# quickwit-oss/quickwit

Hardware: AMD Instinct MI355X
Metric: leaf_search_docs_per_sec (higher is better)
Workload: dtype u32+f32; 1 GPU; 3term_bm25_or_100000000; query=body:w00009 OR body:w00010 OR body:w00011, docs_per_gpu=100000000, splits_per_gpu=1, max_hits=10, parallelism=split-dp1

## Files before the change

### include/quickwit_amd.h

```cpp
#ifndef QUICKWIT_AMD_H
#define QUICKWIT_AMD_H

#include <stddef.h>
#include <stdint.h>

#ifdef __cplusplus
extern "C" {
#endif

typedef struct qw_ctx qw_ctx;

typedef struct qw_buf {
    uint8_t* data;
    size_t len;
} qw_buf;

enum qw_status {
    QW_OK = 0,
    QW_ERR_INVALID_ARGUMENT = -1,
    QW_ERR_INVALID_QUERY = -2,
    QW_ERR_NOT_FOUND = -3,
    QW_ERR_INTERNAL = -4,
    QW_ERR_NO_GPU = -5,
    QW_ERR_BAD_SPLIT = -6,
    QW_ERR_OVER_MEMORY_BUDGET = -7,
};

qw_ctx* qw_ctx_create(const char* config_json);
void qw_ctx_free(qw_ctx* ctx);

int32_t qw_ctx_add_split(qw_ctx* ctx, const char* split_id,
                         const uint8_t* data, size_t len);
int32_t qw_ctx_remove_split(qw_ctx* ctx, const char* split_id);

int32_t qw_leaf_search(qw_ctx* ctx, const uint8_t* leaf_search_request_pb,
                       size_t len, qw_buf* response_pb_out);

void qw_buf_free(qw_buf* buf);

int32_t qw_fetch_docs(qw_ctx* ctx, const uint8_t* fetch_docs_request_pb,
                      size_t len, qw_buf* response_pb_out);

int32_t qw_leaf_list_terms(qw_ctx* ctx, const uint8_t* leaf_list_terms_request_pb,
                           size_t len, qw_buf* response_pb_out);

int32_t qw_merge_leaf_responses(const uint8_t* search_request_pb,
                                size_t search_request_len,
                                const uint8_t** response_pbs,
                                const size_t* response_lens, size_t n,
                                qw_buf* merged_out);

int32_t qw_finalize_agg_to_json(const uint8_t* blob, size_t len,
                                const char* agg_request_json,
                                qw_buf* json_out);

const char* qw_last_error(const qw_ctx* ctx);


int32_t qw_kernel_stats(qw_ctx* ctx, const char* kernel_name,
                        double* total_ms, uint64_t* launches);
void qw_kernel_stats_reset(qw_ctx* ctx);
int32_t qw_ctx_device_sync(qw_ctx* ctx);

int32_t qw_ctx_memory_stats(qw_ctx* ctx, uint64_t* used_bytes,
                            uint64_t* budget_bytes, uint64_t* splits_bytes);

int32_t qw_absence_cache_stats(qw_ctx* ctx, uint64_t* hits, uint64_t* misses,
                               uint64_t* entries);

const char* qw_version(void);

#ifdef __cplusplus
}
#endif

#endif
```

### quickwit_amd/api.py

```python
import ctypes
import json
import os

from . import proto

REPO_ROOT = os.path.dirname(os.path.dirname(os.path.abspath(__file__)))


class _Buf(ctypes.Structure):
    _fields_ = [("data", ctypes.POINTER(ctypes.c_uint8)), ("len", ctypes.c_size_t)]


def _bind(lib, syms):
    getattr(lib, syms["create"]).restype = ctypes.c_void_p
    getattr(lib, syms["add_split"]).argtypes = [
        ctypes.c_void_p, ctypes.c_char_p, ctypes.c_char_p, ctypes.c_size_t]
    getattr(lib, syms["leaf_search"]).argtypes = [
        ctypes.c_void_p, ctypes.c_char_p, ctypes.c_size_t, ctypes.POINTER(_Buf)]
    getattr(lib, syms["last_error"]).restype = ctypes.c_char_p
    getattr(lib, syms["last_error"]).argtypes = [ctypes.c_void_p]
    getattr(lib, syms["buf_free"]).argtypes = [ctypes.POINTER(_Buf)]


class _BaseSearcher:
# ... 98 lines not shown
        buf = _Buf()
        rc = fn(self._ctx, req_pb, len(req_pb), ctypes.byref(buf))
        if rc != 0:
            raise RuntimeError(f"fetch_docs failed ({rc}): {self._err()}")
        out = ctypes.string_at(buf.data, buf.len)
        self._lib.qw_buf_free(ctypes.byref(buf))
        return proto.decode("FetchDocsResponse", out)

    def leaf_list_terms(self, req: dict) -> dict:
        fn = self._lib.qw_leaf_list_terms
        fn.argtypes = [ctypes.c_void_p, ctypes.c_char_p, ctypes.c_size_t,
                       ctypes.POINTER(_Buf)]
        req_pb = proto.encode("LeafListTermsRequest", req)
        buf = _Buf()
        rc = fn(self._ctx, req_pb, len(req_pb), ctypes.byref(buf))
        if rc != 0:
            raise RuntimeError(f"leaf_list_terms failed ({rc}): {self._err()}")
        out = ctypes.string_at(buf.data, buf.len)
        self._lib.qw_buf_free(ctypes.byref(buf))
        return proto.decode("LeafListTermsResponse", out)

    def kernel_stats(self, name: str):
        fn = self._lib.qw_kernel_stats
        fn.argtypes = [ctypes.c_void_p, ctypes.c_char_p,
                       ctypes.POINTER(ctypes.c_double), ctypes.POINTER(ctypes.c_uint64)]
        ms = ctypes.c_double()
        n = ctypes.c_uint64()
        rc = fn(self._ctx, name.encode(), ctypes.byref(ms), ctypes.byref(n))
        if rc != 0:
            raise KeyError(name)
        return ms.value, n.value

    def kernel_stats_reset(self):
        self._lib.qw_kernel_stats_reset.argtypes = [ctypes.c_void_p]
        self._lib.qw_kernel_stats_reset(self._ctx)

    def memory_stats(self):
        fn = self._lib.qw_ctx_memory_stats
        fn.argtypes = [ctypes.c_void_p] + [ctypes.POINTER(ctypes.c_uint64)] * 3
        u, b, s = ctypes.c_uint64(), ctypes.c_uint64(), ctypes.c_uint64()
        rc = fn(self._ctx, ctypes.byref(u), ctypes.byref(b), ctypes.byref(s))
        if rc != 0:
            raise RuntimeError(f"memory_stats failed: {rc}")
        return u.value, b.value, s.value

    def absence_cache_stats(self):
        fn = self._lib.qw_absence_cache_stats
        fn.argtypes = [ctypes.c_void_p] + [ctypes.POINTER(ctypes.c_uint64)] * 3
        h, m, e = ctypes.c_uint64(), ctypes.c_uint64(), ctypes.c_uint64()
        rc = fn(self._ctx, ctypes.byref(h), ctypes.byref(m), ctypes.byref(e))
        if rc != 0:
            raise RuntimeError(f"absence_cache_stats failed: {rc}")
        return h.value, m.value, e.value

    def device_sync(self):
        self._lib.qw_ctx_device_sync.argtypes = [ctypes.c_void_p]
        rc = self._lib.qw_ctx_device_sync(self._ctx)
        if rc != 0:
            raise RuntimeError(f"device_sync failed: {self._err()}")


def make_leaf_request(query_ast: dict | str, schema: dict, splits: list,
                      max_hits: int = 10, sort_fields: list | None = None,
                      aggregation: dict | None = None, start_offset: int = 0,
                      start_timestamp: int | None = None,
                      end_timestamp: int | None = None) -> dict:
    sreq = {
        "index_id_patterns": ["bench-index"],
        "query_ast": query_ast if isinstance(query_ast, str) else json.dumps(query_ast),
        "max_hits": max_hits,
        "start_offset": start_offset,
    }
    if sort_fields:
        sreq["sort_fields"] = sort_fields
    if aggregation is not None:
        sreq["aggregation_request"] = json.dumps(aggregation)
    if start_timestamp is not None:
        sreq["start_timestamp"] = start_timestamp
    if end_timestamp is not None:
        sreq["end_timestamp"] = end_timestamp
    offsets = []
    for s in splits:
        if isinstance(s, dict):
            offsets.append(s)
            continue
        sid, ndocs = s[0], s[1]
        e = {"split_id": sid, "num_docs": ndocs}
        if len(s) > 2:
            e["split_footer_start"], e["split_footer_end"] = s[2], s[3]
        offsets.append(e)
    return {
        "search_request": sreq,
        "leaf_requests": [{"doc_mapper_ord": 0, "index_uri_ord": 0,
                           "split_offsets": offsets}],
        "doc_mappers": [json.dumps(schema)],
        "index_uris": ["ram:///bench-index"],
    }
```

### quickwit_amd/csrc/gpu_types.h

```cpp
#pragma once
#include <cstdint>

namespace qw {

#ifndef QW_TILE_DOCS
#define QW_TILE_DOCS 8192
#endif
constexpr uint32_t TILE_DOCS = QW_TILE_DOCS;
constexpr uint32_t TILE_THREADS = 256;
constexpr uint32_t KTAB_LDS_MAX = 4;
constexpr uint32_t AGG_LDS_BUCKETS = 2048;
constexpr uint32_t TOPK_BINS = 4096;

enum TermRole : uint32_t { ROLE_SHOULD = 0, ROLE_MUST = 1, ROLE_MUST_NOT = 2 };

struct TermDev {
    uint32_t role;
    uint32_t grp;
    uint32_t n_blocks;
    uint64_t skip_off;
    uint64_t payload_off;
    uint64_t norms_off;
    float weight;
    uint32_t ktab_idx;
// ... 62 lines not shown
    uint64_t sub_values_off[4];
    uint64_t sub_nulls_off[4];
    uint32_t sub_width[4];
    uint32_t sub_is_i64[4];
    uint32_t c_shift[4];
    uint32_t c_histo;
    uint32_t c_missing;
    double c_interval[4], c_offset[4];
    int64_t c_base[4];
    uint32_t p_si;
    uint64_t p_out;
    int32_t p_k_lo;
    uint32_t p_n_keys;
    uint64_t p_bound_off;
};

struct QueryDev {
    const uint8_t* split;
    const uint8_t* scratch;
    uint8_t* results;
    uint32_t num_docs;
    uint32_t n_tiles;
    uint32_t n_terms;
    uint32_t n_must;
    uint32_t n_must_not;
    uint32_t n_preds;
    uint32_t n_aggs;
    uint32_t msm;
    uint32_t scoring;
    uint32_t match_all;
    uint32_t collect_hits;
    uint32_t sort_asc;
    uint32_t wide_cand;
    uint32_t sort_src;
    uint32_t sort_width;
    uint64_t sort_values_off;
    uint64_t sort_nulls_off;
    uint32_t agg_fast;
    uint32_t agg_nt;
    uint32_t nt_decode;
    uint64_t bitmap_out;
    uint64_t terms_off;
    uint64_t preds_off;
    uint64_t aggs_off;
    uint64_t ktabs_off;
    uint32_t n_ktabs;
    uint32_t _pad_ktab;
    uint64_t norms_stage_off;
    uint64_t tile_counts_off;
    uint64_t cand_count_off;
    uint64_t cand_off;
    uint64_t cand_cap;
    uint64_t hist_off;
};

}
```

### quickwit_amd/csrc/kernels.hip

```cpp
#include <hip/hip_runtime.h>

#include "gpu_types.h"

namespace qw {

#pragma pack(push, 1)
struct SkipEntryDev {
    uint32_t first_doc;
    uint32_t last_doc;
    uint32_t word_off;
    uint8_t id_bits;
    uint8_t tf_bits;
    uint16_t count;
};
#pragma pack(pop)

__device__ __forceinline__ uint32_t lane_id() { return threadIdx.x & 63u; }

__device__ __forceinline__ uint64_t extract_bits(const uint32_t* base, uint64_t bitpos,
                                                 uint32_t w) {
    uint64_t word = bitpos >> 5;
    uint32_t sh = uint32_t(bitpos & 31);
    uint64_t v = (uint64_t(base[word]) | (uint64_t(base[word + 1]) << 32)) >> sh;
    return v & ((1ull << w) - 1ull);
}

__device__ __forceinline__ void extract_bits_pair(const uint32_t* base, uint32_t j,
                                                  uint32_t w, uint32_t* g0,
                                                  uint32_t* g1) {
    if (w <= 16) {
        uint64_t bitpos = uint64_t(j) * w;
        uint64_t word = bitpos >> 5;
        uint32_t sh = uint32_t(bitpos & 31);
        uint64_t v = (uint64_t(base[word]) | (uint64_t(base[word + 1]) << 32)) >> sh;
        uint32_t mask = (1u << w) - 1u;
        *g0 = uint32_t(v) & mask;
        *g1 = uint32_t(v >> w) & mask;
    } else {
        *g0 = uint32_t(extract_bits(base, uint64_t(j) * w, w));
        *g1 = uint32_t(extract_bits(base, uint64_t(j + 1) * w, w));
    }
}

__device__ __forceinline__ uint32_t wave_incl_scan_u32(uint32_t v) {
    #pragma unroll
    for (int d = 1; d < 64; d <<= 1) {
        uint32_t n = __shfl_up(v, d, 64);
        if ((threadIdx.x & 63u) >= uint32_t(d)) v += n;
    }
    return v;
}

__device__ __forceinline__ uint32_t f32_sortable(float f) {
    uint32_t b = __float_as_uint(f);
    return (b & 0x80000000u) ? ~b : (b | 0x80000000u);
}

__device__ __forceinline__ uint64_t f64_sortable(double d) {
    uint64_t b = __double_as_longlong(d);
    return (b & 0x8000000000000000ull) ? ~b : (b | 0x8000000000000000ull);
}

template <bool NS, bool NB, bool NA, bool NC>
struct SmemMap {
    static constexpr uint32_t score_off = 0;
    static constexpr uint32_t score_end = NS ? TILE_DOCS * 4 : 0;
    static constexpr uint32_t bits_acc_off = score_end;
    static constexpr uint32_t bits_not_off = bits_acc_off + (NB ? TILE_DOCS / 8 : 0);
    static constexpr uint32_t bits_end = bits_not_off + (NB ? TILE_DOCS / 8 : 0);
    static constexpr uint32_t bits_m_off = bits_end;
    static constexpr uint32_t word_pref_off = bits_m_off + (NC ? TILE_DOCS / 8 : 0);
    static constexpr uint32_t coll_end = word_pref_off + (NC ? TILE_DOCS / 8 : 0);
    static constexpr uint32_t agg_hist_off = coll_end;
    static constexpr uint32_t agg_terms_off = agg_hist_off + (NA ? AGG_LDS_BUCKETS * 4 : 0);
    static constexpr uint32_t agg_end = agg_terms_off + (NA ? AGG_LDS_BUCKETS * 4 : 0);
    static constexpr uint32_t tail_off = agg_end;
    static constexpr uint32_t total = tail_off + 4 * 4 + 4 * 4 + 4;
};

constexpr uint32_t tile_lds_bytes(bool ns, bool nb, bool na, bool nc) {
    return (ns ? TILE_DOCS * 4 : 0) + (nb ? 2 * TILE_DOCS / 8 : 0) +
           (nc ? 2 * TILE_DOCS / 8 : 0) + (na ? 2 * AGG_LDS_BUCKETS * 4 : 0) + 36;
}

template <bool SCORE>
__device__ void decode_term_tile(const QueryDev& q, const TermDev& t, uint32_t tile,
                                 uint32_t tile_lo, uint32_t tile_hi, float* score,
                                 uint32_t* bitset, bool scoring,
                                 const float* ktab_lds = nullptr,
                                 const uint8_t* norms_lds = nullptr) {
    const uint32_t* ranges = (const uint32_t*)t.ranges_addr;
    uint32_t blo = ranges[tile], bhi = ranges[q.n_tiles + tile];
    if (blo >= bhi) return;
    const SkipEntryDev* __restrict__ skip = (const SkipEntryDev*)(q.split + t.skip_off);
    const uint32_t* __restrict__ payload = (const uint32_t*)(q.split + t.payload_off);
    const uint8_t* __restrict__ norms = t.norms_off ? q.split + t.norms_off : nullptr;
    const bool nlds = norms_lds && t.norms_off &&
                      t.norms_off == q.norms_stage_off;
    const float* __restrict__ ktab =
        (ktab_lds ? ktab_lds : (const float*)(q.scratch + q.ktabs_off)) +
        256 * t.ktab_idx;
// ... 264 lines not shown
        else lo = mid + 1;
    }
    return lo + 1;
}

__device__ __forceinline__ uint64_t agg_ord(const QueryDev& q, uint64_t values_off,
                                            uint32_t width, uint32_t doc) {
    const uint8_t* col = q.split + values_off;
    switch (width) {
        case 1: return col[doc];
        case 2: return ((const uint16_t*)col)[doc];
        default: return ((const uint32_t*)col)[doc];
    }
}

__device__ __forceinline__ uint64_t wide_sort_key(const QueryDev& q, uint32_t d,
                                                  float sc) {
    if (q.sort_src == 0) return 0;
    if (q.sort_nulls_off) {
        const uint64_t* nulls = (const uint64_t*)(q.split + q.sort_nulls_off);
        if (!((nulls[d >> 6] >> (d & 63)) & 1)) return 0;
    }
    uint64_t S = 0;
    if (q.sort_src == 1) {
        S = uint64_t(f32_sortable(sc)) << 32;
    } else {
        const uint8_t* col = q.split + q.sort_values_off;
        switch (q.sort_width) {
            case 1: S = col[d]; break;
            case 2: S = ((const uint16_t*)col)[d]; break;
            case 4: S = ((const uint32_t*)col)[d]; break;
            default: S = ((const uint64_t*)col)[d]; break;
        }
        if (q.sort_src == 3) S ^= (1ull << 63);
        else if (q.sort_src == 4) S = f64_sortable(__longlong_as_double(S));
    }
    return q.sort_asc ? ~S : S;
}

__device__ __forceinline__ int64_t histo_bucket(const QueryDev& q, const AggDev& a,
                                                uint32_t doc) {
    if (a.int_fast) {
        const int64_t* col = (const int64_t*)(q.split + a.values_off);
        int64_t num = col[doc] - a.i_offset;
        int64_t idx = int64_t(floor(double(num) * a.inv_interval));
        if (idx * a.i_interval > num) --idx;
        else if ((idx + 1) * a.i_interval <= num) ++idx;
        return idx - a.base_index;
    }
    double v = agg_value(q, a.values_off, a.value_width, a.value_is_i64, doc);
    return int64_t(floor((v - a.offset) / a.interval)) - a.base_index;
}

template <bool NS, bool NB, bool NA, bool NC>
__global__ void __launch_bounds__(TILE_THREADS) k_leaf_tile_t(QueryDev q,
                                                              uint32_t tile_base,
                                                              uint32_t tile_end,
                                                              uint32_t do_count) {
    using M = SmemMap<NS, NB, NA, NC>;
    extern __shared__ uint8_t smem[];
    float* sc_score = (float*)(smem + M::score_off);
    uint32_t* sc_bits_acc = (uint32_t*)(smem + M::bits_acc_off);
    uint32_t* sc_bits_not = (uint32_t*)(smem + M::bits_not_off);
    uint32_t* sc_bits_m = (uint32_t*)(smem + M::bits_m_off);
    uint32_t* sc_word_pref = (uint32_t*)(smem + M::word_pref_off);
    uint32_t* sc_agg_hist = (uint32_t*)(smem + M::agg_hist_off);
    uint32_t* sc_agg_terms = (uint32_t*)(smem + M::agg_terms_off);
    uint32_t* sc_agg_matched = (uint32_t*)(smem + M::tail_off);
    uint32_t* sc_wave_base = sc_agg_matched + 4;
    uint32_t* sc_cand_base = sc_wave_base + 4;
    uint8_t* sc_norms = nullptr;
    float* sc_ktabs = nullptr;
    if (NS) {
        uint32_t soff = M::total;
        if (q.norms_stage_off) {
            sc_norms = smem + soff;
            soff += TILE_DOCS;
        }
        if (q.scoring && q.n_ktabs) {
            sc_ktabs = (float*)(smem + soff);
            const float* g = (const float*)(q.scratch + q.ktabs_off);
            for (uint32_t i = threadIdx.x; i < 256u * q.n_ktabs;
                 i += TILE_THREADS)
                sc_ktabs[i] = g[i];
        }
    }

    const TermDev* __restrict__ terms = (const TermDev*)(q.scratch + q.terms_off);
    const PredDev* __restrict__ preds = (const PredDev*)(q.scratch + q.preds_off);
    const AggDev* __restrict__ aggs = (const AggDev*)(q.scratch + q.aggs_off);
    uint32_t* tile_counts = (uint32_t*)(q.results + q.tile_counts_off);
    uint32_t* cand_count = (uint32_t*)(q.results + q.cand_count_off);
    uint64_t* cand = (uint64_t*)(q.results + q.cand_off);

    if (NA && q.n_aggs) {
        for (uint32_t i = threadIdx.x; i < AGG_LDS_BUCKETS; i += TILE_THREADS) {
            sc_agg_hist[i] = 0;
            sc_agg_terms[i] = 0;
        }
        if (threadIdx.x < 4) sc_agg_matched[threadIdx.x] = 0;
    }
    const int64_t* af_col = nullptr;
    const uint8_t* af_tcol = nullptr;
    int64_t af_ioff = 0, af_ivl = 1, af_base = 0;
    double af_inv = 0;
    uint32_t af_twidth = 0, af_hrep = 0, af_trep = 0, af_par = 0;
    bool af_terms = false;
// ... 358 lines not shown
                            if (a.lds_slot == 0)
                                atomicAdd(&sc_agg_hist[a.lds_rep == 2
                                                           ? uint32_t(idx) * 2 +
                                                                 (lane_id() & 1u)
                                                           : uint32_t(idx)],
                                          1u);
                            else
                                atomicAdd((unsigned long long*)(q.results + a.counts_out) +
                                              idx, 1ull);
                            for (uint32_t si = 0; si < a.n_sub; ++si) {
                                if (!a.sub_width[si]) continue;
                                if (a.sub_nulls_off[si]) {
                                    const uint64_t* sn =
                                        (const uint64_t*)(q.split + a.sub_nulls_off[si]);
                                    if (!((sn[d >> 6] >> (d & 63)) & 1)) continue;
                                }
                                double sv = agg_value(q, a.sub_values_off[si],
                                                      a.sub_width[si], a.sub_is_i64[si], d);
                                if (si == a.p_si) {
                                    uint32_t sj = perc_slot(q, a, sv);
                                    atomicAdd((unsigned long long*)(q.results +
                                                                    a.p_out) +
                                                  uint64_t(idx) *
                                                      (a.p_n_keys + 1) +
                                                  sj,
                                              1ull);
                                    continue;
                                }
                                uint8_t* slot = q.results + a.sub_out +
                                                (uint64_t(idx) * a.n_sub + si) * 40;
                                atomicAdd((unsigned long long*)slot, 1ull);
                                atomicAdd((double*)(slot + 8), sv);
                                atomicMin((unsigned long long*)(slot + 16),
                                          (unsigned long long)f64_sortable(sv));
                                atomicMax((unsigned long long*)(slot + 24),
                                          (unsigned long long)f64_sortable(sv));
                                atomicAdd((double*)(slot + 32), sv * sv);
                            }
                        }
                    }
            }
            if (NC) {
                uint64_t mb = __ballot(m);
                uint32_t wbase = (li - lane_id()) >> 5;
                if (lane_id() == 0) sc_bits_m[wbase] = uint32_t(mb);
                else if (lane_id() == 32) sc_bits_m[wbase + 1] = uint32_t(mb >> 32);
            }
        }
        if (NC && q.bitmap_out) {
            __syncthreads();
            ((uint32_t*)q.bitmap_out)[uint64_t(tile) * (TILE_DOCS / 32) +
                                      threadIdx.x] = sc_bits_m[threadIdx.x];
        }
        if (NC) {
            static_assert(TILE_DOCS == 32 * TILE_THREADS,
                          "collection assumes one 32-doc bitset word per thread");
            __syncthreads();
            uint32_t w = threadIdx.x;
            uint32_t cnt = __popc(sc_bits_m[w]);
            uint32_t incl = wave_incl_scan_u32(cnt);
            uint32_t wv = threadIdx.x >> 6;
            if (lane_id() == 63) sc_wave_base[wv] = incl;
            __syncthreads();
            uint32_t wave_off = 0;
            for (uint32_t i = 0; i < wv; ++i) wave_off += sc_wave_base[i];
            sc_word_pref[w] = wave_off + incl - cnt;
            uint32_t tile_total = sc_wave_base[0] + sc_wave_base[1] +
                                  sc_wave_base[2] + sc_wave_base[3];
            if (threadIdx.x == 0) {
                *sc_cand_base = atomicAdd(cand_count, tile_total);
                if (do_count) tile_counts[tile] = tile_total;
            }
            __syncthreads();
            uint64_t base = *sc_cand_base;
            {
                uint32_t wd = threadIdx.x;
                uint32_t bits = sc_bits_m[wd];
                uint64_t rank = sc_word_pref[wd];
                while (bits) {
                    uint32_t b = __ffs(bits) - 1u;
                    bits &= bits - 1u;
                    uint32_t li = wd * 32u + b;
                    uint32_t d = tile_lo + li;
                    float sc = (NS && q.scoring) ? sc_score[li] : 0.f;
                    uint64_t pos = base + rank++;
                    if (pos >= q.cand_cap) break;
                    if (q.wide_cand) {
                        uint64_t key = wide_sort_key(q, d, sc);
                        cand[2 * pos] = key;
                        cand[2 * pos + 1] =
                            (uint64_t(__float_as_uint(sc)) << 32) | d;
                    } else {
                        uint32_t kh = q.scoring ? f32_sortable(sc) : 0u;
                        if (q.sort_asc) kh = ~kh;
                        uint32_t kl = q.sort_asc ? ~d : d;
                        cand[pos] = (uint64_t(kh) << 32) | kl;
                    }
                }
            }
        } else if (do_count) {
            __syncthreads();
            #pragma unroll
            for (int dlt = 32; dlt; dlt >>= 1) local_count += __shfl_down(local_count, dlt, 64);
            if (lane_id() == 0) sc_wave_base[threadIdx.x >> 6] = local_count;
            __syncthreads();
            if (threadIdx.x == 0)
                tile_counts[tile] = sc_wave_base[0] + sc_wave_base[1] +
                                    sc_wave_base[2] + sc_wave_base[3];
        }
        __syncthreads();
    }

    if (NA && q.n_aggs) {
        __syncthreads();
        for (uint32_t ai = 0; ai < q.n_aggs; ++ai) {
            const AggDev& a = aggs[ai];
            if (a.lds_slot > 1) continue;
            uint32_t* src = a.lds_slot == 1 ? sc_agg_terms : sc_agg_hist;
            uint32_t rot = (blockIdx.x * 131u) % (a.n_buckets ? a.n_buckets : 1u);
            for (uint32_t i0 = threadIdx.x; i0 < a.n_buckets;
                 i0 += TILE_THREADS) {
                uint32_t i = i0 + rot;
                if (i >= a.n_buckets) i -= a.n_buckets;
                uint32_t v = a.lds_rep == 2 ? src[2 * i] + src[2 * i + 1] : src[i];
                if (v)
                    atomicAdd((unsigned long long*)(q.results + a.counts_out) + i,
                              (unsigned long long)v);
            }
        }
        if (threadIdx.x < q.n_aggs && threadIdx.x < 4) {
            const AggDev& a = aggs[threadIdx.x];
            if ((a.kind == AGGD_TERMS || a.kind == AGGD_TERMS_NUM) &&
                sc_agg_matched[threadIdx.x])
                atomicAdd((unsigned long long*)(q.results + a.matched_out),
                          (unsigned long long)sc_agg_matched[threadIdx.x]);
        }
    }
}

inline uint32_t launch_leaf_tile(bool ns, bool nb, bool na, bool nc, dim3 grid,
                                 hipStream_t stream, const QueryDev& q,
                                 uint32_t tile_base, uint32_t tile_end,
                                 uint32_t do_count) {
    uint32_t lds = tile_lds_bytes(ns, nb, na, nc);
    if (ns && q.norms_stage_off) lds += TILE_DOCS;
    if (ns && q.scoring && q.n_ktabs) lds += 1024 * q.n_ktabs;
    #define QW_CASE(NS_, NB_, NA_, NC_)                                           \
        if (ns == NS_ && nb == NB_ && na == NA_ && nc == NC_) {                   \
            hipLaunchKernelGGL((k_leaf_tile_t<NS_, NB_, NA_, NC_>), grid,         \
                               dim3(TILE_THREADS), lds, stream, q, tile_base,     \
                               tile_end, do_count);                               \
            return lds;                                                           \
        }
    QW_CASE(false, false, false, false)
    QW_CASE(false, false, false, true)
    QW_CASE(false, false, true, false)
    QW_CASE(false, false, true, true)
    QW_CASE(false, true, false, false)
    QW_CASE(false, true, false, true)
    QW_CASE(false, true, true, false)
    QW_CASE(false, true, true, true)
    QW_CASE(true, false, false, false)
    QW_CASE(true, false, false, true)
    QW_CASE(true, false, true, false)
    QW_CASE(true, false, true, true)
    QW_CASE(true, true, false, false)
    QW_CASE(true, true, false, true)
    QW_CASE(true, true, true, false)
    QW_CASE(true, true, true, true)
    #undef QW_CASE
    return 0;
}

extern "C" __global__ void k_bitmap_combine(uint32_t* dst, const uint32_t* src,
                                            uint64_t words, uint32_t op) {
    for (uint64_t i = blockIdx.x * blockDim.x + threadIdx.x; i < words;
         i += uint64_t(gridDim.x) * blockDim.x) {
        uint32_t d = dst[i], s = src[i];
        switch (op) {
            case 0: d &= s; break;
            case 1: d |= s; break;
            case 2: d &= ~s; break;
            default: d = s; break;
        }
        dst[i] = d;
    }
}

extern "C" __global__ void k_cand_hist(const uint64_t* cand, const uint32_t* n_ptr,
                                       uint64_t prefix, uint32_t prefix_bits,
                                       uint32_t* hist) {
    __shared__ uint32_t lh[TOPK_BINS];
    for (uint32_t i = threadIdx.x; i < TOPK_BINS; i += blockDim.x) lh[i] = 0;
    __syncthreads();
    uint32_t n = *n_ptr;
    uint32_t shift = 64 - prefix_bits - 12;
    uint32_t last_bin = 0xFFFFFFFFu, acc = 0;
    for (uint32_t i = blockIdx.x * blockDim.x + threadIdx.x; i < n;
         i += gridDim.x * blockDim.x) {
        uint64_t k = cand[i];
        if (prefix_bits && (k >> (64 - prefix_bits)) != prefix) continue;
        uint32_t b = uint32_t(k >> shift) & (TOPK_BINS - 1);
        if (b == last_bin) ++acc;
        else {
// ... 223 lines not shown
```

### quickwit_amd/csrc/product.cpp

```cpp
#include <hip/hip_runtime.h>
#include <zlib.h>

#include <algorithm>
#include <chrono>
#include <cmath>
#include <cstdint>
#include <cstdlib>
#include <cstring>
#include <functional>
#include <list>
#include <map>
#include <memory>
#include <set>
#include <stdexcept>
#include <string>
#include <vector>

#include "../../include/quickwit_amd.h"
#include "fieldnorm.h"
#include "minijson.h"
#include "pb.h"
#include "qagg_format.h"
#include "qast.h"
#include "qsplit.h"
// ... 208 lines not shown
                bytes -= it->size;
                idx.erase(it->key);
                it = lru.erase(it);
            } else ++it;
        }
    }
    void clear() {
        for (auto& e : lru) (void)hipFree(e.bm);
        lru.clear();
        idx.clear();
        bytes = 0;
    }
};

}

struct AbsenceCache {
    std::set<std::string> keys;
    uint64_t hits = 0, misses = 0;
    size_t cap = 1 << 20;
    static std::string key(const std::string& split_id, const std::string& f,
                           const std::string& t) {
        std::string k = split_id;
        k += '\0';
        k += f;
        k += '\x1f';
        k += t;
        return k;
    }
    void remove_split(const std::string& split_id) {
        std::string lo = split_id + '\0';
        std::string hi = split_id + '\x01';
        keys.erase(keys.lower_bound(lo), keys.lower_bound(hi));
    }
};

struct qw_ctx {
    int device = 0;
    bool device_ready = false;
    int64_t agg_bucket_limit = 65000;
    std::map<std::string, std::unique_ptr<qw::DeviceSplit>> splits;
    qw::LeafCache leaf_cache;
    qw::HitsetCache hitsets;
    AbsenceCache absence;
    std::string last_error;
    hipStream_t stream = nullptr;
    hipEvent_t ev_start = nullptr, ev_stop = nullptr;
    qw::DevBuf d_scratch, d_results, d_survivors, d_cand2;
    qw::PinnedBuf h_scratch, h_counts, h_surv, h_topk, h_agg;
    std::map<std::string, qw::KernelTimer> timers;
    uint64_t hbm_used = 0;
    uint64_t hbm_budget = 0;
    bool budget_configured = false;
};

static void qw_check_budget(qw_ctx* ctx, uint64_t need) {
    uint64_t used = ctx->hbm_used + ctx->hitsets.bytes;
    if (ctx->hbm_budget && used + need > ctx->hbm_budget)
        throw std::runtime_error(
            "HBM memory budget exceeded: used " + std::to_string(used) +
            " + need " + std::to_string(need) + " > budget " +
            std::to_string(ctx->hbm_budget) +
            " (search_permit_provider analog; raise hbm_memory_budget or "
            "remove splits)");
}

static void qw_ensure_acct(qw_ctx* ctx, qw::DevBuf& b, size_t n) {
    if (n <= b.cap) return;
    qw_check_budget(ctx, n - b.cap);
    ctx->hbm_used -= b.cap;
    b.ensure(n);
    ctx->hbm_used += b.cap;
}

static uint64_t term_ranges_addr(qw_ctx* ctx, const qw::DeviceSplit& ds,
                                 const qw::TextFieldView* f, int64_t tid,
                                 uint32_t n_tiles, uint32_t num_docs) {
    using namespace qw;
    auto key = std::make_pair((const void*)f, tid);
    auto it = ds.range_cache.find(key);
    if (it != ds.range_cache.end()) return (uint64_t)it->second;
    if (ds.range_cache.size() >= 1024) {
        ctx->hbm_used -= ds.range_cache_bytes;
        ds.free_range_cache();
    }
    size_t bytes = 2ull * n_tiles * 4;
    qw_check_budget(ctx, bytes);
    std::vector<uint32_t> r(2ull * n_tiles);
    const SkipEntry* sk = f->h_skip + f->h_skip_off[tid] / 16;
    uint32_t nb = f->h_n_blocks[tid];
    uint32_t* lo = r.data();
    uint32_t* hi = lo + n_tiles;
    uint32_t b_lo = 0, b_hi = 0;
    for (uint32_t tile = 0; tile < n_tiles; ++tile) {
        uint32_t tlo = tile * TILE_DOCS;
        uint32_t thi = std::min<uint32_t>(tlo + TILE_DOCS, num_docs);
        while (b_lo < nb && sk[b_lo].last_doc < tlo) ++b_lo;
        if (b_hi < b_lo) b_hi = b_lo;
        while (b_hi < nb && sk[b_hi].first_doc < thi) ++b_hi;
        lo[tile] = b_lo;
        hi[tile] = b_hi;
    }
    uint8_t* d = nullptr;
    HIP_CHECK(hipMalloc(&d, bytes));
    HIP_CHECK(hipMemcpy(d, r.data(), bytes, hipMemcpyHostToDevice));
    ctx->hbm_used += bytes;
// ... 1408 lines not shown
                      order1 == 0)
                         ? 1
                         : 0;
        q.wide_cand = wide ? 1 : 0;
        if (wide) {
            const SortSpec& s0 = specs[0];
            if (s0.comp == SortSpec::SCORE) {
                q.sort_src = 1;
            } else if (s0.ff) {
                const FastFieldView* f = s0.ff;
                if (f->multi)
                    throw std::runtime_error(
                        "sort by a multi-valued fast field not supported");
                q.sort_values_off = f->values.off;
                q.sort_nulls_off = f->nullable ? f->nulls.off : 0;
                if (f->type == FastFieldView::STR) {
                    q.sort_src = 2;
                    q.sort_width = uint32_t(f->ord_width);
                } else {
                    q.sort_src = f->type == FastFieldView::U64    ? 2
                                 : f->type == FastFieldView::MIXED ? 2
                                 : f->type == FastFieldView::F64  ? 4
                                                                  : 3;
                    q.sort_width = 8;
                }
            } else {
                q.sort_src = 0;
            }
        }
        q.terms_off = off_terms;
        q.preds_off = off_preds;
        q.aggs_off = off_aggs;
        q.ktabs_off = off_ktabs;
        if (fq.scoring) {
            static const bool want_norms = getenv("QW_LDS_NORMS") != nullptr;
            static const bool want_ktab = getenv("QW_LDS_KTAB") != nullptr;
            uint64_t common = 0;
            bool uniform = true;
            for (const TermDev& t : terms)
                if (t.norms_off) {
                    if (!common) common = t.norms_off;
                    else if (common != t.norms_off) uniform = false;
                }
            q.norms_stage_off = (want_norms && uniform) ? common : 0;
            q.n_ktabs = (want_ktab && ktab_fields.size() <= KTAB_LDS_MAX)
                            ? uint32_t(ktab_fields.size())
                            : 0;
        }
        q.tile_counts_off = r_tile_counts;
        q.cand_count_off = r_cand_count;
        q.cand_off = r_cand;
        q.cand_cap = cand_cap;
        q.hist_off = r_hist;

        const char* kname = !fq.terms.empty() ? "union_bm25"
                            : do_aggs         ? "column_agg"
                                              : "range_filter";
        uint32_t n_should = uint32_t(terms.size()) - n_must - n_must_not;
        bool ns = n_should > 0 || (fq.scoring && !terms.empty());
        bool nb = n_must > 0 || n_must_not > 0;
        bool na = do_aggs && !ap.devs.empty();
        uint32_t grid = n_tiles;
        if (na)
            grid = fq.terms.empty()
                       ? std::min<uint32_t>(
                             {n_tiles, 2048u,
                              std::max<uint32_t>(256u, n_tiles / 8)})
                       : std::min<uint32_t>(n_tiles, 2048u);
        if (na && !ap.devs.empty() && ap.devs[0].kind == AGGD_HISTO &&
            ap.devs[0].lds_slot == 0 && ap.devs[0].int_fast &&
            ap.devs[0].n_sub == 0 && ap.devs[0].nulls_off == 0 &&
            ap.devs.size() <= 2 &&
            (ap.devs.size() < 2 ||
             (ap.devs[1].kind == AGGD_TERMS && ap.devs[1].lds_slot == 1 &&
              ap.devs[1].nulls_off == 0 && ap.devs[1].offsets_off == 0 &&
              ap.devs[1].n_buckets > 0)))
            q.agg_fast = 1;
        if (na && ap.devs.size() == 1 && ap.devs[0].kind == AGGD_TERMS &&
            ap.devs[0].lds_slot == 1 && ap.devs[0].n_sub == 0 &&
            ap.devs[0].nulls_off == 0 && ap.devs[0].offsets_off == 0 &&
            ap.devs[0].n_buckets > 0)
            q.agg_fast = 1;
        static const bool agg_nt = getenv("QW_AGG_NT") != nullptr;
        q.agg_nt = agg_nt ? 1 : 0;
        static const bool nt_decode = getenv("QW_NT_DECODE") != nullptr;
        q.nt_decode = nt_decode ? 1 : 0;
        HIP_CHECK(hipEventRecord(ctx->ev_start, ctx->stream));
        launch_leaf_tile(ns, nb, na, collect, dim3(grid), ctx->stream, q, 0u,
                         n_tiles, 1u);
        HIP_CHECK(hipEventRecord(ctx->ev_stop, ctx->stream));
        HIP_CHECK(hipGetLastError());

        bool hist0_valid = false;
        if (collect && !after) {
            uint64_t* d_cand0 = (uint64_t*)(ctx->d_results.p + r_cand);
            uint32_t* d_hist0 = (uint32_t*)(ctx->d_results.p + r_hist);
            uint32_t* d_n0 = (uint32_t*)(ctx->d_results.p + r_cand_count);
            HIP_CHECK(hipMemsetAsync(d_hist0, 0, TOPK_BINS * 4, ctx->stream));
            uint32_t hgrid =
                std::min<uint32_t>(512, (sv.num_docs + 4095) / 4096);
            if (wide)
                hipLaunchKernelGGL(k_cand_hist_w, dim3(hgrid), dim3(256), 0,
                                   ctx->stream, d_cand0, d_n0, 0ull, 0u, d_hist0);
            else
                hipLaunchKernelGGL(k_cand_hist, dim3(hgrid), dim3(256), 0,
                                   ctx->stream, d_cand0, d_n0, 0ull, 0u, d_hist0);
            HIP_CHECK(hipMemcpyAsync(hist0, d_hist0, TOPK_BINS * 4,
                                     hipMemcpyDeviceToHost, ctx->stream));
            hist0_valid = true;
        }

        ctx->h_counts.ensure(size_t(n_tiles) * 4 + 64);
        uint32_t* tile_counts = (uint32_t*)ctx->h_counts.p;
        uint32_t* pc = (uint32_t*)(ctx->h_counts.p + size_t(n_tiles) * 4);
        HIP_CHECK(hipMemcpyAsync(tile_counts, ctx->d_results.p + r_tile_counts,
                                 size_t(n_tiles) * 4, hipMemcpyDeviceToHost,
                                 ctx->stream));
        if (collect)
            HIP_CHECK(hipMemcpyAsync(pc, ctx->d_results.p + r_cand_count, 4,
                                     hipMemcpyDeviceToHost, ctx->stream));
        if (do_aggs && ap.out_bytes) {
            ctx->h_agg.ensure(ap.out_bytes + 64);
            HIP_CHECK(hipMemcpyAsync(ctx->h_agg.p, ctx->d_results.p + r_agg,
                                     ap.out_bytes, hipMemcpyDeviceToHost,
                                     ctx->stream));
        }
        HIP_CHECK(hipStreamSynchronize(ctx->stream));
        uint32_t cand_n = collect ? *pc : 0;
        mark("main+pass0+sync");
        float ms = 0;
        HIP_CHECK(hipEventElapsedTime(&ms, ctx->ev_start, ctx->ev_stop));
        record_kernel_time(ctx, kname, ms);
        for (uint32_t i = 0; i < n_tiles; ++i) matched += tile_counts[i];

        if (collect && cand_n > 0) {
            uint32_t rw = wide ? 2 : 1;
            uint64_t* d_cand = (uint64_t*)(ctx->d_results.p + r_cand);
            uint32_t* d_hist = (uint32_t*)(ctx->d_results.p + r_hist);
            uint32_t* d_scount = (uint32_t*)(ctx->d_results.p + r_cand_count) + 1;
            if (after) {
                uint64_t ceil_key = ~0ull;
                const SortKey& k1 = ck1.key;
                if (wide) {
                    if (!k1.has) ceil_key = 0;
                    else {
                        uint64_t S = k1.key;
                        if (!specs.empty() && specs[0].comp == SortSpec::SCORE) {
                            uint32_t kh = f32_sortable_h(float(u64_to_f64(S)));
                            S = (uint64_t(kh) << 32) | 0xFFFFFFFFull;
                        } else if (!specs.empty() && specs[0].ff &&
                                   specs[0].ff->type == FastFieldView::DATETIME) {
                            int64_t ns = u64_to_i64(S);
                            int64_t ms = ns / 1000000 - ((ns % 1000000) < 0 ? 1 : 0);
                            S = i64_to_u64(ms);
                        }
                        ceil_key = (order1 == 0) ? ~S : S;
                    }
                } else {
                    uint32_t kh = 0;
                    if (fq.scoring && k1.has)
                        kh = f32_sortable_h(float(u64_to_f64(k1.key)));
                    bool nasc = !specs.empty() &&
                                specs[0].comp != SortSpec::DOC_ID && order1 == 0;
                    if (nasc) kh = ~kh;
                    ceil_key = (uint64_t(kh) << 32) | 0xFFFFFFFFull;
                }
                qw_ensure_acct(ctx, ctx->d_cand2, size_t(cand_n) * 8 * rw + 16);
                uint32_t* d_c2n = (uint32_t*)(ctx->d_results.p + r_cand_count) + 2;
                HIP_CHECK(hipMemsetAsync(d_c2n, 0, 4, ctx->stream));
                uint32_t pgrid = std::min<uint32_t>(2048, (cand_n + 255) / 256);
                if (wide)
                    hipLaunchKernelGGL(k_cand_compact_w, dim3(pgrid), dim3(256), 0,
                                       ctx->stream, d_cand, cand_n, 0ull, ceil_key,
                                       (uint64_t*)ctx->d_cand2.p, d_c2n, cand_n);
                else
                    hipLaunchKernelGGL(k_cand_compact, dim3(pgrid), dim3(256), 0,
                                       ctx->stream, d_cand, cand_n, 0ull, ceil_key,
                                       (uint64_t*)ctx->d_cand2.p, d_c2n, cand_n);
                uint32_t n2 = 0;
                HIP_CHECK(hipMemcpyAsync(&n2, d_c2n, 4, hipMemcpyDeviceToHost,
                                         ctx->stream));
                HIP_CHECK(hipStreamSynchronize(ctx->stream));
                d_cand = (uint64_t*)ctx->d_cand2.p;
                cand_n = n2;
            }
        }
// ... 516 lines not shown
static bool is_simple_all_query(const pb::SearchRequest& r) {
    if (r.aggregation_request) return false;
    if (r.search_after) return false;
    if (r.start_timestamp || r.end_timestamp) return false;
    try {
        mj::ValuePtr v = mj::parse(r.query_ast);
        const mj::Value* t = v->get("type");
        return t && t->kind == mj::Value::STR && t->s == "match_all";
    } catch (...) {
        return false;
    }
}

static void disable_search_request_hits(pb::SearchRequest& r) {
    r.max_hits = 0;
    r.start_offset = 0;
    r.sort_fields.clear();
    r.search_after.reset();
}

}

static thread_local std::string g_tls_error;

static void set_err(qw_ctx* ctx, const std::string& msg) {
    if (ctx) ctx->last_error = msg;
    else g_tls_error = msg;
}

static void fill_buf(qw_buf* out, const std::string& s) {
    out->data = (uint8_t*)malloc(s.size() ? s.size() : 1);
    memcpy(out->data, s.data(), s.size());
    out->len = s.size();
}

extern "C" {

const char* qw_version(void) { return "quickwit_amd 0.1 gfx950"; }

qw_ctx* qw_ctx_create(const char* config_json) {
    auto* ctx = new qw_ctx();
    try {
        if (config_json && *config_json) {
            mj::ValuePtr cfg = mj::parse(config_json);
            if (const mj::Value* d = cfg->get("device")) ctx->device = int(d->as_i64());
            if (const mj::Value* b = cfg->get("aggregation_bucket_limit"))
                ctx->agg_bucket_limit = b->as_i64();
            if (const mj::Value* c = cfg->get("partial_request_cache_capacity"))
                ctx->leaf_cache.capacity = size_t(c->as_i64());
            if (const mj::Value* mb = cfg->get("hbm_memory_budget")) {
                ctx->hbm_budget = uint64_t(mb->as_i64());
                ctx->budget_configured = true;
            }
        }
        return ctx;
    } catch (const std::exception& e) {
        g_tls_error = e.what();
        delete ctx;
        return nullptr;
    }
}

void qw_ctx_free(qw_ctx* ctx) {
    if (!ctx) return;
    if (ctx->device_ready) {
        (void)hipSetDevice(ctx->device);
        for (auto& kv : ctx->splits) {
            kv.second->free_range_cache();
            for (auto& sg : kv.second->segs) sg->free_range_cache();
            if (kv.second->d_image) (void)hipFree(kv.second->d_image);
        }
        ctx->hitsets.clear();
        if (ctx->ev_start) (void)hipEventDestroy(ctx->ev_start);
        if (ctx->ev_stop) (void)hipEventDestroy(ctx->ev_stop);
        if (ctx->stream) (void)hipStreamDestroy(ctx->stream);
    }
    delete ctx;
}

const char* qw_last_error(const qw_ctx* ctx) {
    return ctx ? ctx->last_error.c_str() : g_tls_error.c_str();
}

int32_t qw_ctx_add_split(qw_ctx* ctx, const char* split_id, const uint8_t* data,
                         size_t len) {
    using namespace qw;
    try {
        ctx_ensure_device(ctx);
    } catch (const std::exception& e) {
        set_err(ctx, e.what());
        return QW_ERR_NO_GPU;
    }
    try {
        auto ds = std::make_unique<DeviceSplit>();
        ds->host.assign(data, data + len);
        if (len >= 88 && memcmp(data, "QWAMDSP2", 8) == 0) {
            if (memcmp(data + len - 8, "QWA1FOOT", 8) != 0)
                throw std::runtime_error("bad QWA2 footer");
            uint64_t moff, mlen;
            memcpy(&moff, data + len - 24, 8);
            memcpy(&mlen, data + len - 16, 8);
            if (moff + mlen > len) throw std::runtime_error("bad QWA2 footer");
            mj::ValuePtr meta = mj::parse((const char*)data + moff, mlen);
            uint32_t ord = 0;
            for (auto& sgv : meta->at("segments")->arr) {
                uint64_t off = uint64_t(sgv->at("off")->as_i64());
// ... 542 lines not shown
    try {
        IntermediateAggResults ir = IntermediateAggResults::decode(blob, len);
        std::vector<AggDef> defs = parse_agg_request(agg_request_json);
        fill_buf(json_out, finalize_aggs_json(ir, defs));
        return QW_OK;
    } catch (const std::exception& e) {
        set_err(nullptr, e.what());
        return QW_ERR_INTERNAL;
    }
}

int32_t qw_kernel_stats(qw_ctx* ctx, const char* kernel_name, double* total_ms,
                        uint64_t* launches) {
    auto it = ctx->timers.find(kernel_name);
    if (it == ctx->timers.end()) {
        static const char* known[] = {"union_bm25", "range_filter", "column_agg",
                                      "topk_select"};
        bool ok = false;
        for (const char* k : known) ok |= kernel_name == std::string(k);
        if (!ok) return QW_ERR_NOT_FOUND;
        *total_ms = 0;
        *launches = 0;
        return QW_OK;
    }
    *total_ms = it->second.total_ms;
    *launches = it->second.launches;
    return QW_OK;
}

void qw_kernel_stats_reset(qw_ctx* ctx) { ctx->timers.clear(); }

int32_t qw_ctx_memory_stats(qw_ctx* ctx, uint64_t* used_bytes,
                            uint64_t* budget_bytes, uint64_t* splits_bytes) {
    if (!ctx) return QW_ERR_INVALID_ARGUMENT;
    if (used_bytes) *used_bytes = ctx->hbm_used + ctx->hitsets.bytes;
    if (budget_bytes) *budget_bytes = ctx->hbm_budget;
    if (splits_bytes) {
        uint64_t sb = 0;
        for (auto& kv : ctx->splits) sb += kv.second->len + 64;
        *splits_bytes = sb;
    }
    return QW_OK;
}

int32_t qw_absence_cache_stats(qw_ctx* ctx, uint64_t* hits, uint64_t* misses,
                               uint64_t* entries) {
    if (!ctx) return QW_ERR_INVALID_ARGUMENT;
    if (hits) *hits = ctx->absence.hits;
    if (misses) *misses = ctx->absence.misses;
    if (entries) *entries = uint64_t(ctx->absence.keys.size());
    return QW_OK;
}

int32_t qw_ctx_device_sync(qw_ctx* ctx) {
    try {
        ctx_ensure_device(ctx);
        HIP_CHECK(hipDeviceSynchronize());
        return QW_OK;
    } catch (const std::exception& e) {
        set_err(ctx, e.what());
        return QW_ERR_NO_GPU;
    }
}

}
```

Measured before the change: 157.2 billion docs/s.

## Prune top-k candidates in tile kernel using a global running k-th bound

Adds a pruned candidate-collection path to the tile kernel. Each wave sorts its per-thread maximum keys with a bitonic shuffle sort and takes the k-th largest as a local bound. The block then folds that bound into a global atomicMax threshold, and only candidates at or above the threshold are written out. The aim is to cut the candidate volume that later histogram and selection passes have to process for small max_hits, at the cost of extra per-tile sorting, two key evaluations per doc, and an atomic per tile. Adds a config flag and stats counters.

```diff
diff --git a/include/quickwit_amd.h b/include/quickwit_amd.h
--- a/include/quickwit_amd.h
+++ b/include/quickwit_amd.h
@@ -68,6 +68,8 @@
 int32_t qw_absence_cache_stats(qw_ctx* ctx, uint64_t* hits, uint64_t* misses,
                                uint64_t* entries);
 
+int32_t qw_topk_stats(qw_ctx* ctx, uint64_t out[4]);
+
 const char* qw_version(void);
 
 #ifdef __cplusplus
diff --git a/quickwit_amd/api.py b/quickwit_amd/api.py
--- a/quickwit_amd/api.py
+++ b/quickwit_amd/api.py
@@ -174,6 +174,15 @@
         if rc != 0:
             raise RuntimeError(f"absence_cache_stats failed: {rc}")
         return h.value, m.value, e.value
+
+    def topk_stats(self):
+        fn = self._lib.qw_topk_stats
+        fn.argtypes = [ctypes.c_void_p, ctypes.POINTER(ctypes.c_uint64 * 4)]
+        out = (ctypes.c_uint64 * 4)()
+        rc = fn(self._ctx, ctypes.byref(out))
+        if rc != 0:
+            raise RuntimeError(f"topk_stats failed: {rc}")
+        return tuple(out)
 
     def device_sync(self):
         self._lib.qw_ctx_device_sync.argtypes = [ctypes.c_void_p]
diff --git a/quickwit_amd/csrc/gpu_types.h b/quickwit_amd/csrc/gpu_types.h
--- a/quickwit_amd/csrc/gpu_types.h
+++ b/quickwit_amd/csrc/gpu_types.h
@@ -138,6 +138,11 @@
     uint64_t cand_off;
     uint64_t cand_cap;
     uint64_t hist_off;
+    uint32_t prune_k;
+    uint32_t _pad_prune;
 };
 
+constexpr uint32_t TOPK_BOUND_OFF = 16;
+constexpr uint32_t TOPK_PRUNE_MAX_K = 64;
+
 }
diff --git a/quickwit_amd/csrc/kernels.hip b/quickwit_amd/csrc/kernels.hip
--- a/quickwit_amd/csrc/kernels.hip
+++ b/quickwit_amd/csrc/kernels.hip
@@ -47,6 +47,21 @@
     for (int d = 1; d < 64; d <<= 1) {
         uint32_t n = __shfl_up(v, d, 64);
         if ((threadIdx.x & 63u) >= uint32_t(d)) v += n;
+    }
+    return v;
+}
+
+__device__ __forceinline__ uint64_t wave_sort_desc_u64(uint64_t v) {
+    const uint32_t lane = threadIdx.x & 63u;
+    #pragma unroll 1
+    for (uint32_t k = 2; k <= 64; k <<= 1) {
+        #pragma unroll 1
+        for (uint32_t j = k >> 1; j > 0; j >>= 1) {
+            uint64_t o = (uint64_t(__shfl_xor(uint32_t(v >> 32), int(j), 64)) << 32) |
+                         __shfl_xor(uint32_t(v), int(j), 64);
+            bool keep_max = ((lane & j) == 0) == ((lane & k) == 0);
+            v = keep_max ? (v > o ? v : o) : (v < o ? v : o);
+        }
     }
     return v;
 }
@@ -417,7 +432,7 @@
     return int64_t(floor((v - a.offset) / a.interval)) - a.base_index;
 }
 
-template <bool NS, bool NB, bool NA, bool NC>
+template <bool NS, bool NB, bool NA, bool NC, bool PR = false>
 __global__ void __launch_bounds__(TILE_THREADS) k_leaf_tile_t(QueryDev q,
                                                               uint32_t tile_base,
                                                               uint32_t tile_end,
@@ -882,9 +897,9 @@
             ((uint32_t*)q.bitmap_out)[uint64_t(tile) * (TILE_DOCS / 32) +
                                       threadIdx.x] = sc_bits_m[threadIdx.x];
         }
-        if (NC) {
-            static_assert(TILE_DOCS == 32 * TILE_THREADS,
-                          "collection assumes one 32-doc bitset word per thread");
+        static_assert(TILE_DOCS == 32 * TILE_THREADS,
+                      "collection assumes one 32-doc bitset word per thread");
+        if constexpr (NC && !PR) {
             __syncthreads();
             uint32_t w = threadIdx.x;
             uint32_t cnt = __popc(sc_bits_m[w]);
@@ -928,6 +943,86 @@
                     }
                 }
             }
+        } else if constexpr (NC) {
+            __syncthreads();
+            uint32_t w = threadIdx.x;
+            const uint32_t wbits = sc_bits_m[w];
+            uint32_t cnt = __popc(wbits);
+            uint32_t wv = threadIdx.x >> 6;
+            auto narrow_key = [&](uint32_t li) -> uint64_t {
+                float sc = (NS && q.scoring) ? sc_score[li] : 0.f;
+                uint32_t d = tile_lo + li;
+                uint32_t kh = q.scoring ? f32_sortable(sc) : 0u;
+                if (q.sort_asc) kh = ~kh;
+                uint32_t kl = q.sort_asc ? ~d : d;
+                return (uint64_t(kh) << 32) | kl;
+            };
+            uint64_t thr;
+            uint32_t ecnt = 0;
+            {
+                uint64_t wmax = 0;
+                for (uint32_t bits = wbits; bits; bits &= bits - 1u) {
+                    uint64_t key = narrow_key(w * 32u + (__ffs(bits) - 1u));
+                    wmax = key > wmax ? key : wmax;
+                }
+                uint64_t srt = wave_sort_desc_u64(wmax);
+                uint32_t kth_hi = __shfl(uint32_t(srt >> 32), int(q.prune_k - 1), 64);
+                uint32_t kth_lo = __shfl(uint32_t(srt), int(q.prune_k - 1), 64);
+                if (lane_id() == 0) {
+                    sc_word_pref[2 * wv] = kth_hi;
+                    sc_word_pref[2 * wv + 1] = kth_lo;
+                }
+                __syncthreads();
+                if (threadIdx.x == 0) {
+                    uint64_t b = 0;
+                    for (uint32_t i = 0; i < 4; ++i) {
+                        uint64_t wb = (uint64_t(sc_word_pref[2 * i]) << 32) |
+                                      sc_word_pref[2 * i + 1];
+                        b = wb > b ? wb : b;
+                    }
+                    unsigned long long* g = (unsigned long long*)(
+                        q.results + q.cand_count_off + TOPK_BOUND_OFF);
+                    uint64_t old = atomicMax(g, (unsigned long long)b);
+                    uint64_t t = old > b ? old : b;
+                    sc_word_pref[8] = uint32_t(t >> 32);
+                    sc_word_pref[9] = uint32_t(t);
+                }
+                __syncthreads();
+                thr = (uint64_t(sc_word_pref[8]) << 32) | sc_word_pref[9];
+                if (wmax >= thr)
+                    for (uint32_t bits = wbits; bits; bits &= bits - 1u)
+                        ecnt += narrow_key(w * 32u + (__ffs(bits) - 1u)) >= thr;
+            }
+            uint32_t packed = (cnt << 16) | ecnt;
+            uint32_t incl = wave_incl_scan_u32(packed);
+            if (lane_id() == 63) sc_wave_base[wv] = incl;
+            __syncthreads();
+            uint32_t wave_off = 0;
+            for (uint32_t i = 0; i < wv; ++i) wave_off += sc_wave_base[i];
+            sc_word_pref[w] = (wave_off + incl - packed) & 0xFFFFu;
+            uint32_t tile_total = sc_wave_base[0] + sc_wave_base[1] +
+                                  sc_wave_base[2] + sc_wave_base[3];
+            if (threadIdx.x == 0) {
+                *sc_cand_base = atomicAdd(cand_count, tile_total & 0xFFFFu);
+                if (do_count) tile_counts[tile] = tile_total >> 16;
+            }
+            __syncthreads();
+            uint64_t base = *sc_cand_base;
+            if (ecnt) {
+                uint32_t wd = threadIdx.x;
+                uint32_t bits = wbits;
+                uint64_t rank = sc_word_pref[wd];
+                while (bits) {
+                    uint32_t b = __ffs(bits) - 1u;
+                    bits &= bits - 1u;
+                    uint32_t li = wd * 32u + b;
+                    uint64_t key = narrow_key(li);
+                    if (key < thr) continue;
+                    uint64_t pos = base + rank++;
+                    if (pos >= q.cand_cap) break;
+                    cand[pos] = key;
+                }
+            }
         } else if (do_count) {
             __syncthreads();
             #pragma unroll
@@ -975,11 +1070,19 @@
     uint32_t lds = tile_lds_bytes(ns, nb, na, nc);
     if (ns && q.norms_stage_off) lds += TILE_DOCS;
     if (ns && q.scoring && q.n_ktabs) lds += 1024 * q.n_ktabs;
+    const bool pr = q.prune_k != 0;
+    if (pr && (!nc || q.wide_cand || q.prune_k > TOPK_PRUNE_MAX_K))
+        throw std::runtime_error("prune_k needs narrow candidate collection");
     #define QW_CASE(NS_, NB_, NA_, NC_)                                           \
         if (ns == NS_ && nb == NB_ && na == NA_ && nc == NC_) {                   \
-            hipLaunchKernelGGL((k_leaf_tile_t<NS_, NB_, NA_, NC_>), grid,         \
-                               dim3(TILE_THREADS), lds, stream, q, tile_base,     \
-                               tile_end, do_count);                               \
+            if (NC_ && pr)                                                        \
+                hipLaunchKernelGGL((k_leaf_tile_t<NS_, NB_, NA_, NC_, NC_>),      \
+                                   grid, dim3(TILE_THREADS), lds, stream, q,      \
+                                   tile_base, tile_end, do_count);                \
+            else                                                                  \
+                hipLaunchKernelGGL((k_leaf_tile_t<NS_, NB_, NA_, NC_>), grid,     \
+                                   dim3(TILE_THREADS), lds, stream, q, tile_base, \
+                                   tile_end, do_count);                           \
             return lds;                                                           \
         }
     QW_CASE(false, false, false, false)
diff --git a/quickwit_amd/csrc/product.cpp b/quickwit_amd/csrc/product.cpp
--- a/quickwit_amd/csrc/product.cpp
+++ b/quickwit_amd/csrc/product.cpp
@@ -284,6 +284,9 @@
     uint64_t hbm_used = 0;
     uint64_t hbm_budget = 0;
     bool budget_configured = false;
+    bool topk_prune = true;
+    uint64_t topk_pruned = 0, topk_unpruned = 0;
+    uint64_t topk_last_emitted = 0, topk_last_matched = 0;
 };
 
 static void qw_check_budget(qw_ctx* ctx, uint64_t need) {
@@ -1798,6 +1801,11 @@
         q.cand_off = r_cand;
         q.cand_cap = cand_cap;
         q.hist_off = r_hist;
+        uint32_t prune_k = 0;
+        if (collect && !wide && !after && cand_cap > 0 && leaf_max_hits >= 1 &&
+            leaf_max_hits <= TOPK_PRUNE_MAX_K && ctx->topk_prune)
+            prune_k = uint32_t(leaf_max_hits);
+        q.prune_k = prune_k;
 
         const char* kname = !fq.terms.empty() ? "union_bm25"
                             : do_aggs         ? "column_agg"
@@ -1878,6 +1886,11 @@
         HIP_CHECK(hipEventElapsedTime(&ms, ctx->ev_start, ctx->ev_stop));
         record_kernel_time(ctx, kname, ms);
         for (uint32_t i = 0; i < n_tiles; ++i) matched += tile_counts[i];
+        if (collect) {
+            ++(prune_k ? ctx->topk_pruned : ctx->topk_unpruned);
+            ctx->topk_last_emitted = cand_n;
+            ctx->topk_last_matched = matched;
+        }
 
         if (collect && cand_n > 0) {
             uint32_t rw = wide ? 2 : 1;
@@ -2500,6 +2513,9 @@
                 ctx->hbm_budget = uint64_t(mb->as_i64());
                 ctx->budget_configured = true;
             }
+            if (const mj::Value* tp = cfg->get("topk_prune"))
+                ctx->topk_prune = tp->kind == mj::Value::BOOL ? tp->b
+                                                              : tp->as_i64() != 0;
         }
         return ctx;
     } catch (const std::exception& e) {
@@ -3148,6 +3164,15 @@
     return QW_OK;
 }
 
+int32_t qw_topk_stats(qw_ctx* ctx, uint64_t out[4]) {
+    if (!ctx || !out) return QW_ERR_INVALID_ARGUMENT;
+    out[0] = ctx->topk_pruned;
+    out[1] = ctx->topk_unpruned;
+    out[2] = ctx->topk_last_emitted;
+    out[3] = ctx->topk_last_matched;
+    return QW_OK;
+}
+
 int32_t qw_ctx_device_sync(qw_ctx* ctx) {
     try {
         ctx_ensure_device(ctx);
```

Result: faster. 163.7 billion docs/s (median of 6 runs) (+4.1%).
